# DiltheyLab/MetaMaps

Measured on AMD Instinct MI355X. Metric: Gbp long reads mapped+classified per sec (whole node), miniSeq+H DB, higher is better.
Workload: dtype u32

## Files before the change

metamaps_amd/csrc/mm_api.hip:

```cpp
#include "mm_env.hpp"
#include "mm_map.hpp"
#include "mm_em.hpp"
#include "mm_stats.hpp"
#include "mm_synth.hpp"
#include "mm_hpc.hpp"
#include "mm_lca.hpp"
#include "mm_gene.hpp"
#include <chrono>
#include <new>
#include <rccl/rccl.h>
#include <rocprim/rocprim.hpp>

namespace mm {
void seqset_upload(mm_seqset* s);
void seqset_upload_nt16(mm_seqset* s);
int64_t bgzf_inflate(mm_ctx* ctx, const uint8_t* comp, int64_t comp_bytes, const int64_t* comp_off, const int32_t* comp_len, int32_t n,
                     uint8_t* out, int64_t out_cap, const int64_t* out_off, int32_t* status);
void bgzf_deflate(mm_ctx* ctx, const uint8_t* in, int64_t in_bytes, uint8_t* out, int64_t out_cap, int64_t* out_bytes, int32_t* n_blocks);
int64_t bgzf_deflate_bound(int64_t in_bytes);
mm_gzip* gzip_open(mm_ctx* ctx, int64_t chunk, int64_t segment);
void gzip_close(mm_gzip* g);
int gzip_feed(mm_gzip* g, const uint8_t* comp, int64_t n, bool last, int64_t* avail);
int64_t gzip_read(mm_gzip* g, uint8_t* out, int64_t cap);
void gzip_stats(const mm_gzip* g, int64_t* counts, double* seconds);
// ... 273 lines not shown
int64_t mm_hpc_map_device_bytes(const mm_hpc_map* map) { return map ? (int64_t)map->device_bytes() : 0; }
int mm_mapping_to_raw(mm_ctx* ctx, mm_mapping* m, const mm_hpc_map* ref_map, int64_t* end_out, int64_t cap) {
  if (!ctx || !m || !ref_map || cap < 0 || (!end_out && cap > 0)) return MM_ERR_ARG;
  return guarded(ctx, [&] { MM_HIP(hipSetDevice(ctx->device)); mm::mapping_to_raw(ctx, m, ref_map, end_out, cap); });
}
void mm_hpc_map_destroy(mm_hpc_map* map) { if (map) { bind(map->ctx); delete map; } }

int mm_synth_reference(mm_ctx* ctx, const mm_synth_ref_params* p, mm_seqset** out) {
  if (!ctx || !p || !out) return MM_ERR_ARG;
  return guarded(ctx, [&] { MM_HIP(hipSetDevice(ctx->device)); auto* s = new mm_seqset; s->ctx = ctx; try { mm::synth_reference(ctx, *p, s); } catch (...) { delete s; throw; } *out = s; });
}
int mm_synth_community(mm_ctx* ctx, const mm_synth_community_params* p, mm_seqset** out, int32_t* contig_genome) {
  if (!ctx || !p || !out) return MM_ERR_ARG;
  return guarded(ctx, [&] { auto* s = new mm_seqset; s->ctx = ctx; try { mm::synth_community(ctx, *p, s, contig_genome); } catch (...) { delete s; throw; } *out = s; });
}
int mm_synth_community_species(const mm_synth_community_params* p, int32_t* genome_species) {
  if (!p || !genome_species) return MM_ERR_ARG;
  return guarded(nullptr, [&] { mm::synth_community_species(*p, genome_species); });
}
int mm_synth_reads(mm_ctx* ctx, const mm_seqset* reference, const mm_synth_read_params* p, mm_seqset** out, int32_t* truth_genome) {
  if (!ctx || !reference || !p || !out) return MM_ERR_ARG;
  return guarded(ctx, [&] { MM_HIP(hipSetDevice(ctx->device)); auto* s = new mm_seqset; s->ctx = ctx; try { mm::synth_reads(ctx, reference, *p, s, truth_genome); } catch (...) { delete s; throw; } *out = s; });
}

int mm_minimizers(mm_ctx* ctx, const mm_seqset* s, int k, int w, int64_t* offsets, uint32_t* hash, int32_t* wpos, int32_t* strand, int64_t cap) {
  if (!ctx || !s) return MM_ERR_ARG;
  return guarded(ctx, [&] {
    MM_HIP(hipSetDevice(ctx->device));
    mm::MinimizerSet ms;
    mm::run_minimizers(ctx, s, k, w, {}, false, ms);
    if (offsets) for (size_t i = 0; i < ms.h_off.size(); ++i) offsets[i] = (int64_t)ms.h_off[i];
    if (hash || wpos || strand) {
      MM_REQUIRE(cap >= ms.total, MM_ERR_ARG, "output capacity too small");
      auto h = ms.rec.to_host(ctx->stream, (size_t)ms.total);
      for (int64_t i = 0; i < ms.total; ++i) {
        if (hash) hash[i] = h[(size_t)i].hash;
        if (wpos) wpos[i] = mm::pw_wpos(h[(size_t)i].pw);
        if (strand) strand[i] = mm::pw_strand(h[(size_t)i].pw);
      }
    }
  });
}

int mm_index_build(mm_ctx* ctx, const mm_seqset* contigs, int k, int w, mm_index** out) {
  if (!ctx || !contigs || !out) return MM_ERR_ARG;
  return guarded(ctx, [&] {
    MM_HIP(hipSetDevice(ctx->device));
    auto* I = new mm_index;
    try { mm::index_build(ctx, contigs, k, w, I); } catch (...) { delete I; throw; }
    *out = I;
  });
}
int mm_index_plan_chunks(mm_ctx* ctx, const mm_index* whole, uint64_t max_memory_bytes, int32_t* first_contig, int32_t cap, int32_t* n_chunks) {
  if (!ctx || !whole || !n_chunks) return MM_ERR_ARG;
  return guarded(ctx, [&] {
    MM_HIP(hipSetDevice(ctx->device));
    std::vector<int32_t> fc;
    mm::index_plan_chunks(ctx, whole, max_memory_bytes, fc);
    *n_chunks = (int32_t)fc.size();
    if (first_contig) {
      MM_REQUIRE(cap >= (int32_t)fc.size(), MM_ERR_ARG, "output capacity too small");
      for (size_t i = 0; i < fc.size(); ++i) first_contig[i] = fc[i];
    }
  });
}
int mm_index_save(mm_index* idx, const char* path) {
  if (!idx || !path) return MM_ERR_ARG;
// ... 607 lines not shown
```

metamaps_amd/csrc/mm_env.hpp:

```cpp
#pragma once
#include <unistd.h>
#include <cstdlib>
#include <cstring>
#include <string>

extern "C" char** environ;

namespace mm {

struct EnvSwitch { const char* name; const char* dflt; const char* kind; const char* what; };

inline const EnvSwitch* env_table(size_t* n) {
  static const EnvSwitch T[] = {
    {"MM_STRICT_ENV", "unset", "user", "refuse MM_* variables that are not in this table (mm_ctx_create returns MM_ERR_ARG, the CLI exits 1)"},
    {"MM_CPU_BUDGET", "min(hardware threads, affinity mask, cgroup CPU quota)", "user", "CPUs the process may keep busy: what every thread pool of the library and the CLI is sized from (cpu_budget.hpp)"},
    {"MM_SYNC", "block when the CPU budget is <= 32, else spin", "user", "how a host thread waits for its stream: \"spin\" (hipStreamSynchronize) or \"block\" (sleep on an event created with hipEventBlockingSync)"},
    {"MM_CLI_WORKERS", "4", "user", "worker contexts per GPU that take read batches in turn (= --workers-per-gpu)"},
    {"MM_CLI_BATCH_READS", "100000", "user", "reads per batch handed to a worker"},
    {"MM_CLI_BATCH_MBASES", "256", "user", "... or this many million bases, whichever comes first"},
    {"MM_CLI_MAP_SLOTS", "2", "tuning", "batches per device that may be inside their mapping section at the same time"},
    {"MM_CLI_BLOCK_BYTES", "128 MiB", "tuning", "block size of the block-parallel FASTQ/FASTA parser over an mmap-ed query file"},
    {"MM_CLI_REF_BLOCK_BYTES", "min(group, 256 MiB)", "tuning", "the same for the reference FASTA"},
    {"MM_CLI_REF_GROUP_BASES", "2^30", "test", "bases per upload group of the reference (small groups: the concat path on small inputs)"},
    {"MM_CLI_REF_SEQUENTIAL", "unset", "test", "reference through the sequential kseq-style reader instead of the block parser"},
// ... 22 lines not shown
    {"MM_ALLOC_TRACE", "unset", "debug", "every block that comes from the driver, with its cost, on stderr"},
    {"MM_CTX_TRACE", "unset", "debug", "phases of mm_ctx_create (HIP initialisation, stream, allocator) on stderr"},
    {"MM_HOST_TIMING", "unset", "debug", "host-side sections of mm_map_batch and of the index build on stderr"},
    {"MM_PACK_SCALAR", "unset", "test", "mm_seqset_upload packs bases with the byte-table loop only (cross-check of the AVX2 path, host_pack.cpp)"},
    {"MM_INDEX_PART_MAX", "2^31 - 2^24 entries", "test", "entries per partition of the hash sort (small values: the partitioned sort + merge on small inputs)"},
    {"MM_DUP_SAT", "65535", "test", "saturation value of the stored same-hash neighbour distances (small values: K5's scan fall-back)"},
    {"MM_EAGER_TIEBREAK", "unset", "test", "resolve every duplicate-hash strand by the reference's std::sort order up front instead of only where a strand vote reads one"},
    {"MM_FORCE_AMB_REDO", "unset", "test", "every read with an unresolved strand goes through the redo path"},
    {"MM_NO_HIT_FILTER", "unset", "test", "K3 without the exact seed-hit pre-filter: every hit of every kept list reaches the sort (parity tests of the raw hit list)"},
    {"MM_NO_FUSED_FILTER", "unset", "test", "K3 as probe_kernel + two-pass hit_filter_kernel for every read (what reads that do not fit the fused kernel take)"},
    {"MM_HF_STAGE_CAP", "auto", "test", "capacity of a read's survivor stage (tiny values: the overflow / re-filter path)"},
    {"MM_HF_WIDE_FROM", "13000", "tuning", "sketch size from which the two-pass filter counts in 32768 position slots instead of 8192"},
    {"MM_SEGSORT_MAX_KEYS", "2^32 - 1", "test", "keys per call of K4's segmented device sort (small values: the split on small inputs)"},
    {"MM_L1_SERIAL", "unset", "test", "K4's L1 merge loop as the literal one-thread-per-read loop (cross-check of the wavefront form)"},
    {"MM_L2_FULL", "unset", "test", "K5 evaluates every window (the literal slide) instead of the exact skip-ahead"},
    {"MM_L2_DENSE_FROM", "13000", "tuning", "sketch size from which K5 runs as l2_codes_kernel + l2_dense_kernel"},
    {"MM_L2_DENSE_NO_STOP", "unset", "test", "dense path without its early stop (every window evaluated)"},
    {"MM_L2_NO_SMALL_GROUPS", "unset", "test", "groups of fewer than three candidates also run as four-wave workgroups (one launch instead of two)"},
    {"MM_L2_HOST_GROUPS", "unset", "test", "candidate groups formed on the host instead of by l2_group_kernel"},
    {"MM_L2_NO_GROUP_SORT", "unset", "test", "K5 workgroups in read order instead of the order of their candidates' positions"},
    {"MM_L2_GROUP_SORT_MIN", "2048", "tuning", "groups from which the launch order is sorted"},
    {"MM_L2_V1", "unset", "test", "K5's 10 kb class through l2_kernel (rank codes per entry) instead of the zone kernel l2z_kernel (mm_l2z.hpp): the cross-check and the A/B"},
    {"MM_L2_V1_LONG", "unset", "test", "the long-read classes (sketches of 3 073 .. 13 000 hashes) through l2_kernel, the 10 kb class through the zone kernel"},
    {"MM_L2_NO_FUSE", "unset", "test", "zone kernel without the band predicted from L1's seed-hit count: its masks always come from a second pass over the stream"},
    {"MM_L2_NO_RANGES", "unset", "test", "the zone kernel's waves search their candidates' index ranges themselves (until round 6) instead of taking them from l2_ranges_kernel (cross-check)"},
    {"MM_L2Z_FORCE_HANDBACK", "unset", "test", "the zone kernel hands every candidate that reaches its band loop to l2_kernel, as its pass-count guard does (the hand-back path against the default)"},
    {"MM_L2Z_WALK_SEARCH", "unset", "test", "the 10 kb zone kernel finds the next block to sweep by the walk one block at a time (the long-read classes' way) instead of by ballots: the same blocks, the cross-check"},
    {"MM_L2Z_DBG", "unset", "debug", "zone kernel writes pivot-minus-estimate and its pass count INSTEAD OF RESULTS (tools/l2z_pivot_hist.py; 2: against the predicted estimate)"},
    {"MM_L2_ONE_STREAM", "unset", "test", "the two launches of K5's 10 kb class one behind the other on the context's stream instead of side by side (auxiliary stream)"},
    {"MM_L2_NO_SLOTS", "unset", "test", "K5 scratch indexed by wave number of the launch instead of per-XCD slots taken and given back"},
    {"MM_L2_SLOTS", "auto (resident waves)", "tuning", "number of K5 scratch slots"},
    {"MM_L2_STOP", "0", "debug", "K5 leaves after phase n WITHOUT RESULTS (tools/l2_stop.py)"},
    {"MM_L2_PHASES", "unset", "debug", "K5 phase clocks into its counters (tools/l2_long_phases.py; the zone kernel has them in a build with -DL2Z_CLOCKS only)"},
    {"MM_MZ_DBG", "0", "debug", "K1 leaves after step n WITHOUT RESULTS (tools/stage_ms.py)"},
    {"MM_HF_DBG", "0", "debug", "two-pass filter leaves after phase n WITHOUT RESULTS"},
    {"MM_SF_PROF", "unset", "debug", "cycle counts per phase of the streaming seed filter on stderr"},
    {"MM_EM_FORCE_COLLECTIVE", "unset", "test", "a one-rank communicator keeps P1-P3' | ncclAllReduce | finalize instead of P1-P3 alone (how one GPU drives the multi-rank path)"},
    {"MM_EM_GRID", "by size", "tuning", "workgroups of the EM kernels; by default enough for about 160 reads and 448 mappings each, 256 at least, one per read at most; when set: at most 1024 and one per 256 reads"},
    {"MM_GENE_PAIR_BUDGET", "2^26", "test", "(mapping, gene) pairs, feature keys and median keys per tile of mm_gene_overlap (small values: many tiles on small inputs; no result depends on it)"},
    {"MM_GENE_TIMING", "unset", "debug", "device times of mm_gene_overlap's stages (events) on stderr (tools/gene_kernel_stats.py)"},
    {"MM_CLI_FORMAT_PART", "10000", "test", "mapping records per formatter thread of a batch (the text of a batch is formatted in up to eight parts and joined)"},
    {"MM_CLI_CLASSIFY_FROM_FILE", "unset", "test", "mapDirectly --then-classify reads PREFIX back and tokenises it (as `classify` does) instead of taking the lines it has just formatted from memory"},
    {"MM_GATHER_SELF_SEND", "unset", "test", "mm_mapping_gather sends the owner's own parts through ncclSend / ncclRecv too (one-GPU test of the exchange)"},
  };
  *n = sizeof T / sizeof T[0];
  return T;
}

inline std::string env_unknown() {
  size_t n = 0; const EnvSwitch* T = env_table(&n);
  std::string bad;
  for (char** e = environ; e && *e; ++e) {
    if (strncmp(*e, "MM_", 3) != 0) continue;
    const char* eq = strchr(*e, '=');
    const std::string name(*e, eq ? (size_t)(eq - *e) : strlen(*e));
    static const char* const outside[] = {"MM_BENCH_", "MM_FUZZ_", "MM_TEST_", "MM_CLI_FUZZ_CASES", "MM_LIB_PATH"};
    bool ours = false;
    for (const char* pfx : outside) ours = ours || name.rfind(pfx, 0) == 0;
    if (ours) continue;
    bool known = false;
    for (size_t i = 0; i < n && !known; ++i) known = name == T[i].name;
    if (!known) bad += (bad.empty() ? "" : ", ") + name;
  }
  return bad;
}
inline bool env_strict() { const char* e = getenv("MM_STRICT_ENV"); return e && *e && strcmp(e, "0") != 0; }
// ... 3 lines not shown
```

metamaps_amd/csrc/mm_map.hip:

```cpp
#include "mm_map.hpp"
#include <functional>
#include <memory>
#include <rocprim/rocprim.hpp>
#include "mm_l2_core.hpp"
#include "mm_size_classes.hpp"
#include "mm_l2.hpp"
#include "mm_l2z.hpp"
#include "mm_l2_dense.hpp"
#include <cstdlib>
#include <atomic>
#include <thread>
#include "mm_stats.hpp"
#include <algorithm>
#include <numeric>
#include "mm_sketch.hpp"
#include "mm_seed.hpp"
#include "mm_l1.hpp"

namespace mm {

namespace {
struct HostLap {
  const bool on = getenv("MM_HOST_TIMING") != nullptr; std::chrono::steady_clock::time_point t = std::chrono::steady_clock::now();
  void operator()(const char* what) { if (!on) return; const auto n = std::chrono::steady_clock::now(); fprintf(stderr, "host %-28s %8.1f us\n", what, std::chrono::duration<double, std::micro>(n - t).count()); t = n; }
// ... 163 lines not shown
  MapRun(mm_ctx* ctx_, const mm_index* I_, const mm_seqset* reads_, const mm_map_params& P_, mm_mapping* M_)
      : ctx(ctx_), I(I_), reads(reads_), P(P_), M(M_), st(ctx_->stream), T(st), n(reads_->count()) {}

  const std::vector<uint64_t>& hoff() const { return M->mz.h_off; }
  int min_mapped_len() const { return P.w + P.k + 1; }
  bool dense_read(int64_t r, int sr) const { return sr >= sw.dense_from && sr < L2_SKETCH_LIMIT && M->read_len[(size_t)r] >= min_mapped_len(); }
  bool filtering() const { return sw.use_filter && n > 0; }

  void begin() {
    MM_REQUIRE(M->sketch_only || (I && I->k == P.k && I->w == P.w), MM_ERR_ARG, "index was built with different k / window size");
    MM_REQUIRE(n < (1LL << 31), MM_ERR_LIMIT, "more than 2^31 reads in one batch");
    M->ctx = ctx; M->n_reads = n; M->params = P; M->stats = mm_map_stats{};
    M->stats.n_reads = n;
    M->read_len = reads->len;
    M->active.assign((size_t)n, 0);
    for (int64_t r = 0; r < n; ++r) {
      int L = reads->len[(size_t)r];
      bool ok = !(L < P.w || L < P.k || L < P.min_read_len);
      M->active[(size_t)r] = ok;
      if (ok) { M->stats.n_reads_long_enough++; M->stats.bases_long_enough += L; }
    }
    t_total = T.begin(&M->stats.ms_total);
  }

  void minimizers() {
    const mm_mapping* const donor = M->sketch_donor;
    if (donor) {
      const size_t t = T.begin(&M->stats.ms_minimizer);
      auto dcopy = [&](auto& dst, const auto& src) { dst.alloc(src.n); if (src.n) MM_HIP(hipMemcpyAsync(dst.p, src.p, src.bytes(), hipMemcpyDeviceToDevice, st)); };
      mm_mapping* const dn = const_cast<mm_mapping*>(donor);
      const bool same_ctx = donor->ctx == ctx;
      if (same_ctx) M->mz.rec.share_from(dn->mz.rec); else dcopy(M->mz.rec, donor->mz.rec);
      dcopy(M->mz.off, donor->mz.off);
      M->mz.h_off = donor->mz.h_off; M->mz.total = donor->mz.total;
      if (same_ctx) M->sk_hash.share_from(dn->sk_hash); else dcopy(M->sk_hash, donor->sk_hash);
      dcopy(M->sk_strand, donor->sk_strand); dcopy(M->sk_n, donor->sk_n); dcopy(M->amb, donor->amb);
      T.end(t);
    } else { size_t t = T.begin(&M->stats.ms_minimizer); run_minimizers(ctx, reads, P.k, P.w, M->active, false, M->mz); T.end(t); }
    total_mz = M->mz.total;
    if (!donor) {
      M->sk_hash.alloc((size_t)std::max<int64_t>(total_mz, 1));
      M->sk_strand.alloc((size_t)std::max<int64_t>(total_mz, 1));
      M->sk_n.alloc((size_t)std::max<int64_t>(n, 1)); M->sk_n.zero(st);
      M->amb.alloc((size_t)std::max<int64_t>(n, 1)); M->amb.zero(st);
    }
  }

  void sketch() {
    if (M->sketch_donor) return;
    size_t t_sk = T.begin(&M->stats.ms_sketch);
    static_assert(ipt_list_is<4, 6, 8, 10, 12, 16, 20, 24, 32, 40, 48, 64>(SKETCH_IPTS), "the dispatch below lists the classes of mm_size_classes.hpp");
    uint64_t big_seen = 0;
    HostLap hl;
    const ReadBins RB = bin_reads(n, N_SKETCH_CLASSES, [&](int64_t r) -> int {
      const uint64_t c = hoff()[(size_t)r + 1] - hoff()[(size_t)r];
      big_seen |= (uint64_t)(c > SKETCH_LDS_MAX);
      return sketch_class_index(c);
    });
    const bool any_big = big_seen != 0;
    {
      hl("K2 bin");
      DBuf<int32_t> list(std::max<size_t>(RB.order.size(), 1));
      list.upload(RB.order.data(), RB.order.size(), st);
      hl("K2 list upload");
      size_t at = 0;
      for (auto& run : RB.runs) {
        const unsigned nb = (unsigned)run.second;
        const int32_t* lp = list.p + at;
        dispatch<4, 6, 8, 10, 12, 16, 20, 24, 32, 40, 48, 64>(SKETCH_IPTS[run.first], [&](auto ipt_tag) {
          constexpr int IPT = decltype(ipt_tag)::value;
          using SortT = rocprim::block_radix_sort<uint32_t, 256, IPT, uint16_t>;
          using ScanT = rocprim::block_scan<int, 256>;
          const size_t lds = std::max(sizeof(typename SortT::storage_type), sizeof(typename ScanT::storage_type)) + 16;
          if (lds > 48 * 1024) MM_HIP(hipFuncSetAttribute((const void*)sketch_radix_kernel<IPT>, hipFuncAttributeMaxDynamicSharedMemorySize, (int)lds));
          sketch_radix_kernel<IPT><<<dim3(nb), dim3(256), lds, st>>>(M->mz.rec.p, M->mz.off.p, lp, M->sk_hash.p, M->sk_strand.p, M->sk_n.p, M->amb.p);
        });
        MM_KERNEL_CHECK();
        at += run.second;
      }
      hl("K2 launches");
      MM_HIP(mm::stream_sync(st));
      hl("K2 sync (kernels)");
    }
    if (any_big) sketch_big_segmented();
    T.end(t_sk);
  }

  void sketch_big_segmented() {
    std::vector<int32_t> big; std::vector<uint64_t> koff{0};
    for (int64_t r = 0; r < n; ++r) { const uint64_t c = hoff()[(size_t)r + 1] - hoff()[(size_t)r]; if (c > SKETCH_LDS_MAX) { big.push_back((int32_t)r); koff.push_back(koff.back() + c); } }
    const size_t nb = big.size(); const uint64_t nk = koff.back();
    MM_REQUIRE(nk < ((uint64_t)1 << 32), MM_ERR_LIMIT, "more than 2^32 minimizers of reads beyond 16384 minimizers in one batch");
    DBuf<int32_t> d_big(nb); d_big.upload(big.data(), nb, st);
    DBuf<uint64_t> d_koff(nb + 1); d_koff.upload(koff.data(), nb + 1, st);
    DBuf<uint64_t> keys((size_t)nk), sorted((size_t)nk);
    sketch_keys_kernel<<<dim3((unsigned)nb), dim3(256), 0, st>>>(M->mz.rec.p, M->mz.off.p, d_big.p, d_koff.p, keys.p);
    MM_KERNEL_CHECK();
    size_t tmp_bytes = 0;
    MM_HIP(rocprim::segmented_radix_sort_keys(nullptr, tmp_bytes, keys.p, sorted.p, (unsigned int)nk, (unsigned int)nb, d_koff.p, d_koff.p + 1, 0, 64, st));
    DBuf<uint8_t> tmp(std::max<size_t>(tmp_bytes, 16));
    MM_HIP(rocprim::segmented_radix_sort_keys((void*)tmp.p, tmp_bytes, keys.p, sorted.p, (unsigned int)nk, (unsigned int)nb, d_koff.p, d_koff.p + 1, 0, 64, st));
    sketch_finish_kernel<<<dim3((unsigned)nb), dim3(256), 0, st>>>(M->mz.rec.p, M->mz.off.p, d_big.p, d_koff.p, sorted.p, M->sk_hash.p, M->sk_strand.p, M->sk_n.p, M->amb.p);
    MM_KERNEL_CHECK();
    MM_HIP(mm::stream_sync(st));
  }

  bool after_sketch() {
    hl.t = std::chrono::steady_clock::now();
    M->h_sk_n = M->sk_n.to_host(st, (size_t)n);
    if (M->sketch_only) {
      for (int64_t r = 0; r < n; ++r) M->stats.sum_sketch += M->h_sk_n[(size_t)r];
      M->h_rec_off.assign((size_t)n + 1, 0); M->n_rec = 0;
      T.end(t_total);
      T.collect();
      return false;
    }
    if (M->at_stage) M->at_stage(M->at_stage_user, 1);
    h_amb = M->amb.to_host(st, (size_t)n);
    hl("post-K2 downloads");
    int64_t giant = 0;
    for (int64_t r = 0; r < n; ++r) if (M->h_sk_n[(size_t)r] >= L2_SKETCH_LIMIT) ++giant;
    M->stats.n_reads_giant = giant;
    return true;
  }

  void tiebreak_lists() {
    for (int64_t r = 0; r < n; ++r) if (h_amb[(size_t)r]) (sw.eager_tiebreak ? eager_reads : lazy_reads).push_back(r);
    M->stats.n_ambiguous_sketch_reads = (int64_t)(eager_reads.size() + lazy_reads.size());
    hl("post-K2 amb lists");
    if (!eager_reads.empty()) amb_finish = start_tiebreak(eager_reads);
    hl("post-K2 tiebreak start");
  }

  std::function<void()> start_tiebreak(const std::vector<int64_t>& amb_reads) {
    const size_t na = amb_reads.size();
    std::vector<uint64_t> so(na), dof(na + 1, 0);
    std::vector<int32_t> expect(na);
    for (size_t i = 0; i < na; ++i) {
      int64_t r = amb_reads[i];
      so[i] = hoff()[(size_t)r];
      dof[i + 1] = dof[i] + (hoff()[(size_t)r + 1] - hoff()[(size_t)r]);
      expect[i] = M->h_sk_n[(size_t)r];
    }
    DBuf<uint64_t> d_so(na), d_do(na + 1);
    d_so.upload(so.data(), na, st); d_do.upload(dof.data(), na + 1, st);
    DBuf<Rec> comp((size_t)dof[na]);
    gather_amb_kernel<<<dim3((unsigned)na), dim3(256), 0, st>>>(M->mz.rec.p, d_so.p, d_do.p, comp.p);
    MM_KERNEL_CHECK();
    amb_states.push_back(std::make_unique<AmbState>());
    AmbState* const A = amb_states.back().get();
    A->hr = comp.to_host(st);
    A->dof = dof; A->expect = std::move(expect); A->d_so = std::move(d_so); A->d_do = std::move(d_do);
    A->sv.assign((size_t)dof[na], 0);
    A->scnt.assign(na, 0);
    A->bg = std::thread([A, na]() {
      std::atomic<size_t> next{0};
      auto worker = [&]() {
        std::vector<HostMz> v;
        for (size_t i = next.fetch_add(1); i < na; i = next.fetch_add(1)) {
          const size_t cntr = (size_t)(A->dof[i + 1] - A->dof[i]);
          v.resize(cntr);
          for (size_t j = 0; j < cntr; ++j) { const Rec& x = A->hr[(size_t)A->dof[i] + j]; v[j] = HostMz{x.hash, pw_wpos(x.pw), pw_strand(x.pw)}; }
          std::sort(v.begin(), v.end(), host_less_by_hash);
          auto ue = std::unique(v.begin(), v.end(), host_eq_by_hash);
          const size_t sN = (size_t)(ue - v.begin());
          if ((int64_t)sN != A->expect[i]) A->mismatch = 1;
          for (size_t j = 0; j < sN; ++j) A->sv[(size_t)A->dof[i] + j] = v[j].strand == 1 ? 1 : 0;
          A->scnt[i] = (int32_t)sN;
        }
      };
      const unsigned nthr = std::max(1u, std::min(32u, std::min<unsigned>(mm::cpu_budget(), (unsigned)((na + 15) / 16))));
      std::vector<std::thread> pool;
      for (unsigned t = 1; t < nthr; ++t) pool.emplace_back(worker);
      worker();
      for (auto& t : pool) t.join();
    });
    return [M = M, A, na, st = st]() {
      if (A->bg.joinable()) A->bg.join();
      MM_REQUIRE(A->mismatch == 0, MM_ERR_DEVICE, "sketch size disagrees between device and host tie-break");
      DBuf<uint8_t> d_sv(A->sv.size()); d_sv.upload(A->sv.data(), A->sv.size(), st);
// ... 642 lines not shown
```

metamaps_amd/csrc/mm_minimizer.hpp:

```cpp
#pragma once
#include <type_traits>
#include "mm_common.hpp"
#include "mm_scan.hpp"

namespace mm {

constexpr int MZ_THREADS = 256;
constexpr int MZ_TILE = 2048;
constexpr int MZ_MAX_W = 4096;
constexpr int MZ_STAGE = 1024;
constexpr int MZ_MAX_K = 64;

struct SeqView {
  const uint32_t* packed;
  const uint64_t* base;
  const int32_t* len;
  const uint64_t* exc_start;
  const uint32_t* exc_len;
  const uint8_t* exc_byte;
  int64_t n_exc;
  int64_t n;
};

__device__ inline uint32_t code_at(const SeqView& S, uint64_t g) { return (S.packed[g >> 4] >> (2 * (g & 15))) & 3u; }
// ... 305 lines not shown
  for (int i = 0; i < MZ_TILE / MZ_THREADS; ++i) {
    int j = j0 + i, p = H0 + j;
    if (j < np && p >= w - 1 && (flg[j] & 1)) {
      int pj = -1;
      const int qlo = max(max(j - w + 1, 0), (w - 1) - H0);
      for (int q = j - 1; q >= qlo; --q) if (flg[q] & 1) { pj = q; break; }
      bool emit = (pj < 0) || (cps[pj] != cps[j]);
      if (p > w - 1 && p < js) emit = false;
      if (emit) mask |= 1u << i;
    }
  }
  }
  const uint32_t cnt = __popc(mask);
  uint64_t tot;
  uint64_t ex = block_excl_scan_u64(cnt, &tot);
  if (dbgs == 4) { if (MODE != 1 && tid == 0) tile_count[tile] = 0; return; }
  if (MODE != 1 && tid == 0) tile_count[tile] = (uint32_t)tot;
  if (MODE == 2 && tot > MZ_STAGE) { if (tid == 0) atomicExch(stage_overflow, 1); return; }
  if (MODE != 0) {
    uint64_t o = (MODE == 1 ? tile_out[tile] : tile * (uint64_t)MZ_STAGE) + ex;
#pragma unroll
    for (int i = 0; i < MZ_TILE / MZ_THREADS; ++i) {
      if (mask & (1u << i)) {
        int j = j0 + i, p = H0 + j, c = cps[j];
        uint32_t pw = ((uint32_t)(p - w + 1) << PW_SHIFT) | ((flg[c] & 2) ? PW_STRAND : 0u);
        out[o] = Rec{hsh[c], pw};
        if (out_seq) out_seq[o] = (uint32_t)s;
        ++o;
      }
    }
  }
}

static __global__ void __launch_bounds__(256) compact_tiles_kernel(const Rec* __restrict__ stage, const uint32_t* __restrict__ tile_count,
                                                                   const uint64_t* __restrict__ tile_out, Rec* __restrict__ out) {
  const uint64_t tile = blockIdx.x;
  const uint32_t n = tile_count[tile];
  const uint64_t o = tile_out[tile];
  for (uint32_t i = threadIdx.x; i < n; i += 256) out[o + i] = stage[tile * (uint64_t)MZ_STAGE + i];
}

inline size_t minimizer_lds_bytes(int k, int w) {
  int halo = (2 * (w - 1) + 7) & ~7, NP = MZ_TILE + halo, NB = ((NP + k - 1 + 8) + 15) & ~15;
  return (size_t)2 * NB + (size_t)NP * 4 + (size_t)NP * 2 + (size_t)NP;
}

struct MinimizerSet {
  DBuf<Rec> rec;
  DBuf<uint64_t> off;
  DBuf<uint32_t> rec_seq;
  std::vector<uint64_t> h_off;
  int64_t total = 0;
};

void run_minimizers(mm_ctx* ctx, const mm_seqset* S, int k, int w, const std::vector<uint8_t>& active, bool want_rec_seq,
                    MinimizerSet& out);

SeqView make_view(const mm_seqset* S);

}
```

metamaps_amd/csrc/mm_seq.hip:

```cpp
#include "mm_minimizer.hpp"
#include <algorithm>
#include <thread>
#include <atomic>
#include <cstdio>
#include <cstring>

extern "C" int mm_host_has_avx2();
extern "C" size_t mm_pack_acgt_blocks(const uint8_t* p, size_t n_bases, uint32_t* out);

namespace mm {

SeqView make_view(const mm_seqset* S) {
  return SeqView{S->packed.p, S->d_base.p, S->d_len.p, S->exc_start.p, S->exc_len.p, S->exc_byte.p, S->n_exc, S->count()};
}

__global__ void gather_offsets_kernel(const uint64_t* __restrict__ tile_first, const uint64_t* __restrict__ tile_out, int64_t n,
                                      uint64_t* __restrict__ off) {
  int64_t s = (int64_t)blockIdx.x * blockDim.x + threadIdx.x;
  if (s <= n) off[s] = tile_out[tile_first[s]];
}

void run_minimizers(mm_ctx* ctx, const mm_seqset* S, int k, int w, const std::vector<uint8_t>& active, bool want_rec_seq,
                    MinimizerSet& out) {
  MM_REQUIRE(S->frozen, MM_ERR_STATE, "sequence set not uploaded");
// ... 14 lines not shown
  out.total = 0;
  if (ntiles == 0) { out.off.zero(st); out.rec.alloc(0); MM_HIP(mm::stream_sync(st)); return; }
  MM_REQUIRE(ntiles < (1LL << 31), MM_ERR_LIMIT, "too many tiles for one launch");

  DBuf<uint64_t> d_tf((size_t)n + 1);
  d_tf.upload(tf.data(), tf.size(), st);
  DBuf<uint8_t> d_act;
  if (!active.empty()) { d_act.alloc(active.size()); d_act.upload(active.data(), active.size(), st); }
  DBuf<int32_t> d_js((size_t)n);
  SeqView V = make_view(S);
  jstar_kernel<<<dim3((unsigned)ceil_div(n, 128)), dim3(128), 0, st>>>(V, d_act.p, k, w, d_js.p);
  MM_KERNEL_CHECK();

  const size_t lds = minimizer_lds_bytes(k, w);
  if (lds > 64 * 1024) {
    MM_HIP(hipFuncSetAttribute((const void*)minimizer_kernel<0>, hipFuncAttributeMaxDynamicSharedMemorySize, (int)lds));
    MM_HIP(hipFuncSetAttribute((const void*)minimizer_kernel<1>, hipFuncAttributeMaxDynamicSharedMemorySize, (int)lds));
    MM_HIP(hipFuncSetAttribute((const void*)minimizer_kernel<2>, hipFuncAttributeMaxDynamicSharedMemorySize, (int)lds));
  }
  DBuf<uint32_t> tcount((size_t)ntiles);
  DBuf<uint64_t> tout((size_t)ntiles + 1), tmp;
  bool single_pass = !want_rec_seq && (size_t)ntiles * MZ_STAGE * sizeof(Rec) <= ((size_t)6 << 30);
  DBuf<Rec> stage;
  DBuf<int> d_ovf(1); d_ovf.zero(st);
  if (single_pass) {
    stage.alloc((size_t)ntiles * MZ_STAGE);
    { const char* e = getenv("MM_MZ_DBG"); int v = e ? atoi(e) : 0; MM_HIP(hipMemcpyToSymbolAsync(HIP_SYMBOL(mz_dbg_stop), &v, sizeof v, 0, hipMemcpyHostToDevice, st)); }
    minimizer_kernel<2><<<dim3((unsigned)ntiles), dim3(MZ_THREADS), lds, st>>>(V, d_tf.p, k, w, d_js.p, tcount.p, nullptr, stage.p, nullptr, d_ovf.p);
  } else {
    minimizer_kernel<0><<<dim3((unsigned)ntiles), dim3(MZ_THREADS), lds, st>>>(V, d_tf.p, k, w, d_js.p, tcount.p, nullptr, nullptr, nullptr, nullptr);
  }
  MM_KERNEL_CHECK();
  exclusive_scan_u32_u64(tcount.p, ntiles, tout.p, tmp, st);
  uint64_t total = 0;
  int h_ovf = 0;
  MM_HIP(hipMemcpyAsync(&total, tout.p + ntiles, sizeof total, hipMemcpyDeviceToHost, st));
  MM_HIP(hipMemcpyAsync(&h_ovf, d_ovf.p, sizeof h_ovf, hipMemcpyDeviceToHost, st));
  MM_HIP(mm::stream_sync(st));
  if (h_ovf) single_pass = false;
  out.total = (int64_t)total;
  out.rec.alloc((size_t)total);
  if (want_rec_seq) out.rec_seq.alloc((size_t)total);
  if (total) {
    if (single_pass)
      compact_tiles_kernel<<<dim3((unsigned)ntiles), dim3(256), 0, st>>>(stage.p, tcount.p, tout.p, out.rec.p);
    else
      minimizer_kernel<1><<<dim3((unsigned)ntiles), dim3(MZ_THREADS), lds, st>>>(V, d_tf.p, k, w, d_js.p, nullptr, tout.p, out.rec.p,
                                                                               want_rec_seq ? out.rec_seq.p : nullptr, nullptr);
    MM_KERNEL_CHECK();
  }
  gather_offsets_kernel<<<dim3((unsigned)ceil_div(n + 1, 256)), dim3(256), 0, st>>>(d_tf.p, tout.p, n, out.off.p);
  MM_KERNEL_CHECK();
  out.off.download(out.h_off.data(), (size_t)n + 1, st);
  MM_HIP(mm::stream_sync(st));
}

static inline int code_of(uint8_t c) {
  switch (c) { case 'A': return 0; case 'C': return 1; case 'G': return 2; case 'T': return 3; }
  return -1;
}

void seqset_upload(mm_seqset* s) {
  MM_REQUIRE(!s->frozen, MM_ERR_STATE, "sequence set already uploaded");
  hipStream_t st = s->ctx->stream;
  const size_t n = s->staged.size();
  s->len.resize(n);
  s->base.assign(n + 1, 0);
  s->total_bases = 0;
  for (size_t i = 0; i < n; ++i) {
    MM_REQUIRE((int64_t)s->staged[i].second <= MAX_SEQ_LEN, MM_ERR_LIMIT, "sequence longer than 2^29-1 bases");
    s->len[i] = (int32_t)s->staged[i].second;
    s->base[i + 1] = s->base[i] + (((uint64_t)s->len[i] + 15) & ~15ull);
    s->total_bases += s->len[i];
  }
  const size_t nwords = (size_t)(s->base[n] >> 4);
  uint32_t* const words = (uint32_t*)s->ctx->pinned_up_at_least((nwords + 1) * sizeof(uint32_t));
  words[nwords] = 0;
  std::vector<uint64_t> es; std::vector<uint32_t> el; std::vector<uint8_t> eb;
  {
    static const struct Lut { uint8_t t[256]; Lut() { for (int c = 0; c < 256; ++c) { int u = (c > 96 && c < 123) ? c - 32 : c; int k = code_of((uint8_t)u); t[c] = k >= 0 ? (uint8_t)k : 0x80; } } } lut;
    struct Item { size_t seq; size_t j0, j1; };
    struct Runs { std::vector<uint64_t> es; std::vector<uint32_t> el; std::vector<uint8_t> eb; };
    constexpr size_t PIECE = (size_t)4 << 20;
    std::vector<Item> items;
    for (size_t i = 0; i < n; ++i) { const size_t L = s->staged[i].second; for (size_t j0 = 0; j0 < L; j0 += PIECE) items.push_back(Item{i, j0, std::min(L, j0 + PIECE)}); }
    std::vector<Runs> runs(items.size());
    const unsigned hw = mm::cpu_budget();
// ... 427 lines not shown
```

metamaps_amd/csrc/mm_sketch.hpp:

```cpp
#pragma once
#include <rocprim/rocprim.hpp>
#include "mm_map.hpp"

namespace mm {

template <int IPT>
__global__ void __launch_bounds__(256) sketch_radix_kernel(const Rec* __restrict__ rec, const uint64_t* __restrict__ off,
                                                           const int32_t* __restrict__ read_list, uint32_t* __restrict__ sk_hash,
                                                           uint8_t* __restrict__ sk_strand, int32_t* __restrict__ sk_n, uint8_t* __restrict__ amb) {
  using Sort = rocprim::block_radix_sort<uint32_t, 256, IPT, uint16_t>;
  using Scan = rocprim::block_scan<int, 256>;
  union Tmp { typename Sort::storage_type sort; typename Scan::storage_type scan; };
  extern __shared__ __align__(16) unsigned char sketch_dyn[];
  Tmp& tmp = *reinterpret_cast<Tmp*>(sketch_dyn);
  __shared__ uint32_t last_key[256];
  __shared__ uint8_t last_st[256];
  __shared__ int s_amb;
  const int r = read_list[blockIdx.x];
  const uint64_t o = off[r];
  const int n = (int)(off[r + 1] - o);
  const int t = threadIdx.x;
  uint32_t key[IPT]; uint16_t val[IPT];
#pragma unroll
  for (int i = 0; i < IPT; ++i) { const int idx = t * IPT + i; key[i] = idx < n ? rec[o + idx].hash : 0xffffffffu; val[i] = (uint16_t)idx; }
  if (t == 0) s_amb = 0;
  Sort().sort(key, val, tmp.sort);
  uint8_t stv[IPT];
#pragma unroll
  for (int i = 0; i < IPT; ++i) stv[i] = (t * IPT + i < n) ? (uint8_t)(rec[o + val[i]].pw & PW_STRAND) : 0;
  last_key[t] = key[IPT - 1]; last_st[t] = stv[IPT - 1];
  __syncthreads();
  int nfirst = 0; bool first[IPT]; bool ambig = false;
#pragma unroll
  for (int i = 0; i < IPT; ++i) {
    const int pos = t * IPT + i;
    const uint32_t pk = i ? key[i - 1] : (t ? last_key[t - 1] : 0u);
    const uint8_t ps = i ? stv[i - 1] : (t ? last_st[t - 1] : 0);
    first[i] = pos < n && (pos == 0 || pk != key[i]);
    if (pos < n && pos > 0 && pk == key[i] && ps != stv[i]) ambig = true;
    nfirst += first[i] ? 1 : 0;
  }
  if (ambig) s_amb = 1;
  int ex = 0, total = 0;
  Scan().exclusive_scan(nfirst, ex, 0, total, tmp.scan);
  const int ex0 = ex;
#pragma unroll
  for (int i = 0; i < IPT; ++i) if (first[i]) { sk_hash[o + ex] = key[i]; sk_strand[o + ex] = stv[i]; ++ex; }
  __threadfence_block();
  __syncthreads();
  if (s_amb) {
    int ex2 = ex0;
#pragma unroll
    for (int i = 0; i < IPT; ++i) {
      const int pos = t * IPT + i;
      if (first[i]) ++ex2;
      const uint32_t pk = i ? key[i - 1] : (t ? last_key[t - 1] : 0u);
      const uint8_t ps = i ? stv[i - 1] : (t ? last_st[t - 1] : 0);
      if (pos < n && pos > 0 && pk == key[i] && ps != stv[i]) sk_strand[o + ex2 - 1] |= 2;
    }
  }
  if (t == 0) { sk_n[r] = total; amb[r] = (uint8_t)(s_amb ? 2 : 0); }
}

__global__ void __launch_bounds__(256) sketch_keys_kernel(const Rec* __restrict__ rec, const uint64_t* __restrict__ off, const int32_t* __restrict__ read_list,
                                                          const uint64_t* __restrict__ koff, uint64_t* __restrict__ keys) {
  const int r = read_list[blockIdx.x];
  const uint64_t o = off[r], k0 = koff[blockIdx.x];
  const uint32_t n = (uint32_t)(off[r + 1] - o);
  for (uint32_t i = threadIdx.x; i < n; i += 256) keys[k0 + i] = ((uint64_t)rec[o + i].hash << 32) | i;
}
__global__ void __launch_bounds__(256) sketch_finish_kernel(const Rec* __restrict__ rec, const uint64_t* __restrict__ off, const int32_t* __restrict__ read_list,
                                                            const uint64_t* __restrict__ koff, const uint64_t* __restrict__ sorted,
                                                            uint32_t* __restrict__ sk_hash, uint8_t* __restrict__ sk_strand, int32_t* __restrict__ sk_n, uint8_t* __restrict__ amb) {
  const int r = read_list[blockIdx.x];
  const uint64_t o = off[r];
  const uint64_t* __restrict__ a = sorted + koff[blockIdx.x];
  const int n = (int)(off[r + 1] - o);
  __shared__ int s_amb;
  if (threadIdx.x == 0) s_amb = 0;
  __syncthreads();
  for (int pass = 0; pass < 2; ++pass) {
    uint64_t carry = 0;
    for (int base = 0; base < n; base += 256) {
      const int i = base + threadIdx.x;
      bool first = false, differs = false; uint32_t h = 0, stv = 0;
      if (i < n) {
        const uint64_t key = a[i];
        h = (uint32_t)(key >> 32);
        stv = rec[o + (uint32_t)key].pw & PW_STRAND;
        if (i == 0) first = true;
        else {
          const uint64_t pk = a[i - 1];
          first = (uint32_t)(pk >> 32) != h;
          differs = !first && (rec[o + (uint32_t)pk].pw & PW_STRAND) != stv;
        }
      }
      uint64_t tot;
      const uint64_t ex = block_excl_scan_u64(first ? 1 : 0, &tot);
      if (pass == 0) {
        if (first) { sk_hash[o + carry + ex] = h; sk_strand[o + carry + ex] = (uint8_t)stv; }
        if (differs) s_amb = 1;
      } else if (differs) sk_strand[o + carry + ex - 1] |= 2;
      carry += tot;
    }
    __threadfence_block();
    __syncthreads();
    if (pass == 0) {
      if (threadIdx.x == 0) { sk_n[r] = (int32_t)carry; amb[r] = (uint8_t)(s_amb ? 2 : 0); }
      if (!s_amb) break;
    }
  }
}

__global__ void __launch_bounds__(256) gather_amb_kernel(const Rec* __restrict__ rec, const uint64_t* __restrict__ src_off,
                                                         const uint64_t* __restrict__ dst_off, Rec* __restrict__ out) {
  const uint64_t so = src_off[blockIdx.x], d0 = dst_off[blockIdx.x], n = dst_off[blockIdx.x + 1] - d0;
  for (uint64_t i = threadIdx.x; i < n; i += 256) out[d0 + i] = rec[so + i];
}
__global__ void __launch_bounds__(256) scatter_strand_kernel(const uint8_t* __restrict__ in, const uint64_t* __restrict__ src_off,
                                                             const uint64_t* __restrict__ dst_off, const int32_t* __restrict__ cnt,
                                                             uint8_t* __restrict__ sk_strand) {
  const uint64_t d0 = dst_off[blockIdx.x], so = src_off[blockIdx.x];
  const int n = cnt[blockIdx.x];
  for (int i = threadIdx.x; i < n; i += 256) sk_strand[so + i] = in[d0 + i];
}

}
```

Before: 26.05.

## Read minimizers from staged tiles in place instead of compacting them

When the minimizer kernel finishes in a single pass, the staged per-tile records are kept as they are, along with tile offsets. The compaction kernel and the second packed buffer are skipped. Sketch kernels reach records through a tile-aware accessor (SeqRecs) that keeps tile bounds in LDS or searches them in global memory. The strand bit is also carried inside the sort keys and values, so the sketch finish step no longer re-reads the records. The cost is indirection and binary search on each access, extra tile metadata copied between donors, and more memory held by the sparse staged buffer.

```diff
diff --git a/metamaps_amd/csrc/mm_api.hip b/metamaps_amd/csrc/mm_api.hip
--- a/metamaps_amd/csrc/mm_api.hip
+++ b/metamaps_amd/csrc/mm_api.hip
@@ -329,7 +329,7 @@
     if (offsets) for (size_t i = 0; i < ms.h_off.size(); ++i) offsets[i] = (int64_t)ms.h_off[i];
     if (hash || wpos || strand) {
       MM_REQUIRE(cap >= ms.total, MM_ERR_ARG, "output capacity too small");
-      auto h = ms.rec.to_host(ctx->stream, (size_t)ms.total);
+      auto h = mm::minimizer_records_to_host(ctx, ms);
       for (int64_t i = 0; i < ms.total; ++i) {
         if (hash) hash[i] = h[(size_t)i].hash;
         if (wpos) wpos[i] = mm::pw_wpos(h[(size_t)i].pw);
diff --git a/metamaps_amd/csrc/mm_env.hpp b/metamaps_amd/csrc/mm_env.hpp
--- a/metamaps_amd/csrc/mm_env.hpp
+++ b/metamaps_amd/csrc/mm_env.hpp
@@ -78,6 +78,7 @@
     {"MM_L2_SLOTS", "auto (resident waves)", "tuning", "number of K5 scratch slots"},
     {"MM_L2_STOP", "0", "debug", "K5 leaves after phase n WITHOUT RESULTS (tools/l2_stop.py)"},
     {"MM_L2_PHASES", "unset", "debug", "K5 phase clocks into its counters (tools/l2_long_phases.py; the zone kernel has them in a build with -DL2Z_CLOCKS only)"},
+    {"MM_MZ_COMPACT", "unset", "test", "1: the staged tiles of a read batch's minimizers are packed back to back (compact_tiles_kernel) before K2 instead of read where K1 staged them (cross-check of the staged layout and its A/B partner)"},
     {"MM_MZ_DBG", "0", "debug", "K1 leaves after step n WITHOUT RESULTS (tools/stage_ms.py)"},
     {"MM_HF_DBG", "0", "debug", "two-pass filter leaves after phase n WITHOUT RESULTS"},
     {"MM_SF_PROF", "unset", "debug", "cycle counts per phase of the streaming seed filter on stderr"},
diff --git a/metamaps_amd/csrc/mm_map.hip b/metamaps_amd/csrc/mm_map.hip
--- a/metamaps_amd/csrc/mm_map.hip
+++ b/metamaps_amd/csrc/mm_map.hip
@@ -219,6 +219,7 @@
       const bool same_ctx = donor->ctx == ctx;
       if (same_ctx) M->mz.rec.share_from(dn->mz.rec); else dcopy(M->mz.rec, donor->mz.rec);
       dcopy(M->mz.off, donor->mz.off);
+      dcopy(M->mz.tout, donor->mz.tout); dcopy(M->mz.tile_first, donor->mz.tile_first);
       M->mz.h_off = donor->mz.h_off; M->mz.total = donor->mz.total;
       if (same_ctx) M->sk_hash.share_from(dn->sk_hash); else dcopy(M->sk_hash, donor->sk_hash);
       dcopy(M->sk_strand, donor->sk_strand); dcopy(M->sk_n, donor->sk_n); dcopy(M->amb, donor->amb);
@@ -260,7 +261,7 @@
           using ScanT = rocprim::block_scan<int, 256>;
           const size_t lds = std::max(sizeof(typename SortT::storage_type), sizeof(typename ScanT::storage_type)) + 16;
           if (lds > 48 * 1024) MM_HIP(hipFuncSetAttribute((const void*)sketch_radix_kernel<IPT>, hipFuncAttributeMaxDynamicSharedMemorySize, (int)lds));
-          sketch_radix_kernel<IPT><<<dim3(nb), dim3(256), lds, st>>>(M->mz.rec.p, M->mz.off.p, lp, M->sk_hash.p, M->sk_strand.p, M->sk_n.p, M->amb.p);
+          sketch_radix_kernel<IPT><<<dim3(nb), dim3(256), lds, st>>>(M->mz.store(), lp, M->sk_hash.p, M->sk_strand.p, M->sk_n.p, M->amb.p);
         });
         MM_KERNEL_CHECK();
         at += run.second;
@@ -281,13 +282,13 @@
     DBuf<int32_t> d_big(nb); d_big.upload(big.data(), nb, st);
     DBuf<uint64_t> d_koff(nb + 1); d_koff.upload(koff.data(), nb + 1, st);
     DBuf<uint64_t> keys((size_t)nk), sorted((size_t)nk);
-    sketch_keys_kernel<<<dim3((unsigned)nb), dim3(256), 0, st>>>(M->mz.rec.p, M->mz.off.p, d_big.p, d_koff.p, keys.p);
+    sketch_keys_kernel<<<dim3((unsigned)nb), dim3(256), 0, st>>>(M->mz.store(), d_big.p, d_koff.p, keys.p);
     MM_KERNEL_CHECK();
     size_t tmp_bytes = 0;
     MM_HIP(rocprim::segmented_radix_sort_keys(nullptr, tmp_bytes, keys.p, sorted.p, (unsigned int)nk, (unsigned int)nb, d_koff.p, d_koff.p + 1, 0, 64, st));
     DBuf<uint8_t> tmp(std::max<size_t>(tmp_bytes, 16));
     MM_HIP(rocprim::segmented_radix_sort_keys((void*)tmp.p, tmp_bytes, keys.p, sorted.p, (unsigned int)nk, (unsigned int)nb, d_koff.p, d_koff.p + 1, 0, 64, st));
-    sketch_finish_kernel<<<dim3((unsigned)nb), dim3(256), 0, st>>>(M->mz.rec.p, M->mz.off.p, d_big.p, d_koff.p, sorted.p, M->sk_hash.p, M->sk_strand.p, M->sk_n.p, M->amb.p);
+    sketch_finish_kernel<<<dim3((unsigned)nb), dim3(256), 0, st>>>(M->mz.off.p, d_big.p, d_koff.p, sorted.p, M->sk_hash.p, M->sk_strand.p, M->sk_n.p, M->amb.p);
     MM_KERNEL_CHECK();
     MM_HIP(mm::stream_sync(st));
   }
@@ -322,17 +323,20 @@
   std::function<void()> start_tiebreak(const std::vector<int64_t>& amb_reads) {
     const size_t na = amb_reads.size();
     std::vector<uint64_t> so(na), dof(na + 1, 0);
-    std::vector<int32_t> expect(na);
+    std::vector<int32_t> expect(na), rl(na);
     for (size_t i = 0; i < na; ++i) {
       int64_t r = amb_reads[i];
+      rl[i] = (int32_t)r;
       so[i] = hoff()[(size_t)r];
       dof[i + 1] = dof[i] + (hoff()[(size_t)r + 1] - hoff()[(size_t)r]);
       expect[i] = M->h_sk_n[(size_t)r];
     }
     DBuf<uint64_t> d_so(na), d_do(na + 1);
     d_so.upload(so.data(), na, st); d_do.upload(dof.data(), na + 1, st);
+    DBuf<int32_t> d_rl(na);
+    d_rl.upload(rl.data(), na, st);
     DBuf<Rec> comp((size_t)dof[na]);
-    gather_amb_kernel<<<dim3((unsigned)na), dim3(256), 0, st>>>(M->mz.rec.p, d_so.p, d_do.p, comp.p);
+    gather_amb_kernel<<<dim3((unsigned)na), dim3(256), 0, st>>>(M->mz.store(), d_rl.p, d_do.p, comp.p);
     MM_KERNEL_CHECK();
     amb_states.push_back(std::make_unique<AmbState>());
     AmbState* const A = amb_states.back().get();
diff --git a/metamaps_amd/csrc/mm_minimizer.hpp b/metamaps_amd/csrc/mm_minimizer.hpp
--- a/metamaps_amd/csrc/mm_minimizer.hpp
+++ b/metamaps_amd/csrc/mm_minimizer.hpp
@@ -361,11 +361,10 @@
   }
 }
 
-static __global__ void __launch_bounds__(256) compact_tiles_kernel(const Rec* __restrict__ stage, const uint32_t* __restrict__ tile_count,
-                                                                   const uint64_t* __restrict__ tile_out, Rec* __restrict__ out) {
+static __global__ void __launch_bounds__(256) compact_tiles_kernel(const Rec* __restrict__ stage, const uint64_t* __restrict__ tile_out, Rec* __restrict__ out) {
   const uint64_t tile = blockIdx.x;
-  const uint32_t n = tile_count[tile];
   const uint64_t o = tile_out[tile];
+  const uint32_t n = (uint32_t)(tile_out[tile + 1] - o);
   for (uint32_t i = threadIdx.x; i < n; i += 256) out[o + i] = stage[tile * (uint64_t)MZ_STAGE + i];
 }
 
@@ -373,17 +372,67 @@
   int halo = (2 * (w - 1) + 7) & ~7, NP = MZ_TILE + halo, NB = ((NP + k - 1 + 8) + 15) & ~15;
   return (size_t)2 * NB + (size_t)NP * 4 + (size_t)NP * 2 + (size_t)NP;
 }
+
+struct RecStore {
+  const Rec* rec; const uint64_t* off; const uint64_t* tout; const uint64_t* tile_first;
+};
+
+constexpr int REC_LDS_TILES = 63;
+struct SeqRecs {
+  const Rec* rec;
+  const uint64_t* tb_g;
+  const uint32_t* tb_l;
+  uint64_t t0, o;
+  int nt;
+  bool in_lds;
+  struct Cursor { int t = -1; uint32_t lo = 0, hi = 0; };
+  __device__ SeqRecs(const RecStore& R, int64_t s, uint32_t* lds_tb) {
+    o = R.off[s]; tb_g = nullptr; tb_l = lds_tb; t0 = 0; nt = 0; rec = R.rec + o; in_lds = false;
+    if (R.tout) {
+      t0 = R.tile_first[s]; nt = (int)(R.tile_first[s + 1] - t0);
+      rec = R.rec; tb_g = R.tout + t0;
+      if (lds_tb) {
+        in_lds = nt <= REC_LDS_TILES;
+        if (in_lds) for (int i = threadIdx.x; i <= nt; i += blockDim.x) lds_tb[i] = (uint32_t)(tb_g[i] - o);
+        __syncthreads();
+      }
+    }
+  }
+  __device__ uint32_t bound(int i) const { return in_lds ? tb_l[i] : (uint32_t)(tb_g[i] - o); }
+  __device__ int tile_of(uint32_t idx) const {
+    int lo = 0, hi = nt;
+    while (hi - lo > 1) { const int mid = (lo + hi) >> 1; if (bound(mid) <= idx) lo = mid; else hi = mid; }
+    return lo;
+  }
+  __device__ const Rec& at(uint32_t idx, Cursor& c) const {
+    if (!tb_g) return rec[idx];
+    if (c.t < 0) { c.t = tile_of(idx); c.lo = bound(c.t); c.hi = bound(c.t + 1); }
+    while (idx >= c.hi) { ++c.t; c.lo = c.hi; c.hi = bound(c.t + 1); }
+    return rec[(t0 + (uint64_t)c.t) * MZ_STAGE + (idx - c.lo)];
+  }
+  template <typename F> __device__ void for_each_run(uint32_t n, F&& f) const {
+    if (!tb_g) { f(0u, n, rec); return; }
+    for (int t = 0; t < nt; ++t) {
+      const uint32_t a = bound(t), b = bound(t + 1);
+      if (b > a) f(a, b - a, rec + (t0 + (uint64_t)t) * MZ_STAGE);
+    }
+  }
+};
 
 struct MinimizerSet {
   DBuf<Rec> rec;
   DBuf<uint64_t> off;
   DBuf<uint32_t> rec_seq;
+  DBuf<uint64_t> tout, tile_first;
   std::vector<uint64_t> h_off;
   int64_t total = 0;
+  bool staged() const { return tout.p != nullptr; }
+  RecStore store() const { return RecStore{rec.p, off.p, tout.p, tile_first.p}; }
 };
 
 void run_minimizers(mm_ctx* ctx, const mm_seqset* S, int k, int w, const std::vector<uint8_t>& active, bool want_rec_seq,
                     MinimizerSet& out);
+std::vector<Rec> minimizer_records_to_host(mm_ctx* ctx, const MinimizerSet& ms);
 
 SeqView make_view(const mm_seqset* S);
 
diff --git a/metamaps_amd/csrc/mm_seq.hip b/metamaps_amd/csrc/mm_seq.hip
--- a/metamaps_amd/csrc/mm_seq.hip
+++ b/metamaps_amd/csrc/mm_seq.hip
@@ -70,27 +70,41 @@
   }
   MM_KERNEL_CHECK();
   exclusive_scan_u32_u64(tcount.p, ntiles, tout.p, tmp, st);
-  uint64_t total = 0;
+  gather_offsets_kernel<<<dim3((unsigned)ceil_div(n + 1, 256)), dim3(256), 0, st>>>(d_tf.p, tout.p, n, out.off.p);
+  MM_KERNEL_CHECK();
+  out.off.download(out.h_off.data(), (size_t)n + 1, st);
   int h_ovf = 0;
-  MM_HIP(hipMemcpyAsync(&total, tout.p + ntiles, sizeof total, hipMemcpyDeviceToHost, st));
   MM_HIP(hipMemcpyAsync(&h_ovf, d_ovf.p, sizeof h_ovf, hipMemcpyDeviceToHost, st));
   MM_HIP(mm::stream_sync(st));
   if (h_ovf) single_pass = false;
+  const uint64_t total = out.h_off[(size_t)n];
   out.total = (int64_t)total;
+  out.tout.release(); out.tile_first.release();
+  const char* const e_compact = getenv("MM_MZ_COMPACT");
+  if (single_pass && !(e_compact && e_compact[0] == '1')) {
+    out.rec = std::move(stage); out.tout = std::move(tout); out.tile_first = std::move(d_tf);
+    return;
+  }
   out.rec.alloc((size_t)total);
   if (want_rec_seq) out.rec_seq.alloc((size_t)total);
   if (total) {
     if (single_pass)
-      compact_tiles_kernel<<<dim3((unsigned)ntiles), dim3(256), 0, st>>>(stage.p, tcount.p, tout.p, out.rec.p);
+      compact_tiles_kernel<<<dim3((unsigned)ntiles), dim3(256), 0, st>>>(stage.p, tout.p, out.rec.p);
     else
       minimizer_kernel<1><<<dim3((unsigned)ntiles), dim3(MZ_THREADS), lds, st>>>(V, d_tf.p, k, w, d_js.p, nullptr, tout.p, out.rec.p,
                                                                                want_rec_seq ? out.rec_seq.p : nullptr, nullptr);
     MM_KERNEL_CHECK();
   }
-  gather_offsets_kernel<<<dim3((unsigned)ceil_div(n + 1, 256)), dim3(256), 0, st>>>(d_tf.p, tout.p, n, out.off.p);
+  MM_HIP(mm::stream_sync(st));
+}
+
+std::vector<Rec> minimizer_records_to_host(mm_ctx* ctx, const MinimizerSet& ms) {
+  hipStream_t st = ctx->stream;
+  if (!ms.staged() || ms.total == 0) return ms.rec.to_host(st, (size_t)ms.total);
+  DBuf<Rec> packed((size_t)ms.total);
+  compact_tiles_kernel<<<dim3((unsigned)(ms.tout.n - 1)), dim3(256), 0, st>>>(ms.rec.p, ms.tout.p, packed.p);
   MM_KERNEL_CHECK();
-  out.off.download(out.h_off.data(), (size_t)n + 1, st);
-  MM_HIP(mm::stream_sync(st));
+  return packed.to_host(st);
 }
 
 static inline int code_of(uint8_t c) {
diff --git a/metamaps_amd/csrc/mm_sketch.hpp b/metamaps_amd/csrc/mm_sketch.hpp
--- a/metamaps_amd/csrc/mm_sketch.hpp
+++ b/metamaps_amd/csrc/mm_sketch.hpp
@@ -4,8 +4,9 @@
 
 namespace mm {
 
+static_assert(SKETCH_LDS_MAX <= (1u << 15), "bit 15 of the sort's 16-bit value carries the strand");
 template <int IPT>
-__global__ void __launch_bounds__(256) sketch_radix_kernel(const Rec* __restrict__ rec, const uint64_t* __restrict__ off,
+__global__ void __launch_bounds__(256) sketch_radix_kernel(const RecStore RS,
                                                            const int32_t* __restrict__ read_list, uint32_t* __restrict__ sk_hash,
                                                            uint8_t* __restrict__ sk_strand, int32_t* __restrict__ sk_n, uint8_t* __restrict__ amb) {
   using Sort = rocprim::block_radix_sort<uint32_t, 256, IPT, uint16_t>;
@@ -16,18 +17,25 @@
   __shared__ uint32_t last_key[256];
   __shared__ uint8_t last_st[256];
   __shared__ int s_amb;
+  __shared__ uint32_t s_tb[REC_LDS_TILES + 1];
   const int r = read_list[blockIdx.x];
-  const uint64_t o = off[r];
-  const int n = (int)(off[r + 1] - o);
+  const uint64_t o = RS.off[r];
+  const int n = (int)(RS.off[r + 1] - o);
   const int t = threadIdx.x;
+  const SeqRecs recs(RS, r, s_tb);
   uint32_t key[IPT]; uint16_t val[IPT];
+  SeqRecs::Cursor cur;
 #pragma unroll
-  for (int i = 0; i < IPT; ++i) { const int idx = t * IPT + i; key[i] = idx < n ? rec[o + idx].hash : 0xffffffffu; val[i] = (uint16_t)idx; }
+  for (int i = 0; i < IPT; ++i) {
+    const int idx = t * IPT + i;
+    key[i] = 0xffffffffu; val[i] = (uint16_t)idx;
+    if (idx < n) { const Rec x = recs.at((uint32_t)idx, cur); key[i] = x.hash; val[i] = (uint16_t)(idx | ((x.pw & PW_STRAND) ? 0x8000 : 0)); }
+  }
   if (t == 0) s_amb = 0;
   Sort().sort(key, val, tmp.sort);
   uint8_t stv[IPT];
 #pragma unroll
-  for (int i = 0; i < IPT; ++i) stv[i] = (t * IPT + i < n) ? (uint8_t)(rec[o + val[i]].pw & PW_STRAND) : 0;
+  for (int i = 0; i < IPT; ++i) stv[i] = (t * IPT + i < n) ? (uint8_t)(val[i] >> 15) : 0;
   last_key[t] = key[IPT - 1]; last_st[t] = stv[IPT - 1];
   __syncthreads();
   int nfirst = 0; bool first[IPT]; bool ambig = false;
@@ -62,14 +70,17 @@
   if (t == 0) { sk_n[r] = total; amb[r] = (uint8_t)(s_amb ? 2 : 0); }
 }
 
-__global__ void __launch_bounds__(256) sketch_keys_kernel(const Rec* __restrict__ rec, const uint64_t* __restrict__ off, const int32_t* __restrict__ read_list,
+__global__ void __launch_bounds__(256) sketch_keys_kernel(const RecStore RS, const int32_t* __restrict__ read_list,
                                                           const uint64_t* __restrict__ koff, uint64_t* __restrict__ keys) {
   const int r = read_list[blockIdx.x];
-  const uint64_t o = off[r], k0 = koff[blockIdx.x];
-  const uint32_t n = (uint32_t)(off[r + 1] - o);
-  for (uint32_t i = threadIdx.x; i < n; i += 256) keys[k0 + i] = ((uint64_t)rec[o + i].hash << 32) | i;
+  const uint64_t k0 = koff[blockIdx.x];
+  const uint32_t n = (uint32_t)(RS.off[r + 1] - RS.off[r]);
+  const SeqRecs recs(RS, r, nullptr);
+  recs.for_each_run(n, [&](uint32_t first, uint32_t cnt, const Rec* __restrict__ p) {
+    for (uint32_t i = threadIdx.x; i < cnt; i += 256) { const Rec x = p[i]; keys[k0 + first + i] = ((uint64_t)x.hash << 32) | ((uint64_t)(first + i) << 1) | (x.pw & PW_STRAND); }
+  });
 }
-__global__ void __launch_bounds__(256) sketch_finish_kernel(const Rec* __restrict__ rec, const uint64_t* __restrict__ off, const int32_t* __restrict__ read_list,
+__global__ void __launch_bounds__(256) sketch_finish_kernel(const uint64_t* __restrict__ off, const int32_t* __restrict__ read_list,
                                                             const uint64_t* __restrict__ koff, const uint64_t* __restrict__ sorted,
                                                             uint32_t* __restrict__ sk_hash, uint8_t* __restrict__ sk_strand, int32_t* __restrict__ sk_n, uint8_t* __restrict__ amb) {
   const int r = read_list[blockIdx.x];
@@ -87,12 +98,12 @@
       if (i < n) {
         const uint64_t key = a[i];
         h = (uint32_t)(key >> 32);
-        stv = rec[o + (uint32_t)key].pw & PW_STRAND;
+        stv = (uint32_t)key & 1u;
         if (i == 0) first = true;
         else {
           const uint64_t pk = a[i - 1];
           first = (uint32_t)(pk >> 32) != h;
-          differs = !first && (rec[o + (uint32_t)pk].pw & PW_STRAND) != stv;
+          differs = !first && ((uint32_t)pk & 1u) != stv;
         }
       }
       uint64_t tot;
@@ -112,10 +123,13 @@
   }
 }
 
-__global__ void __launch_bounds__(256) gather_amb_kernel(const Rec* __restrict__ rec, const uint64_t* __restrict__ src_off,
+__global__ void __launch_bounds__(256) gather_amb_kernel(const RecStore RS, const int32_t* __restrict__ read_list,
                                                          const uint64_t* __restrict__ dst_off, Rec* __restrict__ out) {
-  const uint64_t so = src_off[blockIdx.x], d0 = dst_off[blockIdx.x], n = dst_off[blockIdx.x + 1] - d0;
-  for (uint64_t i = threadIdx.x; i < n; i += 256) out[d0 + i] = rec[so + i];
+  const uint64_t d0 = dst_off[blockIdx.x], n = dst_off[blockIdx.x + 1] - d0;
+  const SeqRecs recs(RS, read_list[blockIdx.x], nullptr);
+  recs.for_each_run((uint32_t)n, [&](uint32_t first, uint32_t cnt, const Rec* __restrict__ p) {
+    for (uint32_t i = threadIdx.x; i < cnt; i += 256) out[d0 + first + i] = p[i];
+  });
 }
 __global__ void __launch_bounds__(256) scatter_strand_kernel(const uint8_t* __restrict__ in, const uint64_t* __restrict__ src_off,
                                                              const uint64_t* __restrict__ dst_off, const int32_t* __restrict__ cnt,
```

After: 25.88, median of 2. No clear change (-0.6%).
